# starkware-libs/stark-perpetual

Hardware: AMD Instinct MI355X
Metric: pedersen_hashes_per_sec (higher is better)
Workload: dtype u32x9; 1 GPU; 2^16-leaf Pedersen Merkle rebuild per GPU (BASELINE.json configs[1]), 63 rebuilds in lockstep; tree_height=16, leaves_per_gpu=65536, calls_per_region=28, streams=2, window_bits=26, combine=none

## Files before the change

### stark-perpetual_amd/csrc/curve.hpp

```cpp
#pragma once
#include "fp29.hpp"

namespace sp {

struct aff {
  fe x, y;
};
struct xyzz {
  fe X, Y, ZZ, ZZZ;
};
struct jac {
  fe X, Y, Z;
};

SP_HD xyzz xyzz_from_aff(const aff& p) {
  xyzz r;
  r.X = p.x;
  r.Y = p.y;
  r.ZZ = FE_ONE_M;
  r.ZZZ = FE_ONE_M;
  return r;
}

template <bool SCAN = false>
SP_HD xyzz xyzz_madd(const xyzz& a, const aff& q) {
  if constexpr (SCAN && SP_FE_SCAN) {
    fe t[3];
    fe_scan(t, scan_mul{q.x, a.ZZ}, scan_mul{q.y, a.ZZZ});
    const fe P = fe_sub(t[0], a.X), R = fe_sub(t[1], a.Y);
    const fe P2 = fe_dbl(P), R2 = fe_dbl(R);
    fe_scan(t, scan_sqr{P, P2}, scan_sqr{R, R2});
    const fe PP = t[0], RR = t[1];
    fe_scan(t, scan_mul{P, PP}, scan_mul{a.X, PP});
    const fe PPP = t[0], Q = t[1];
    xyzz r;
    r.X = fe_carry(fe_sub(fe_sub(RR, PPP), fe_dbl(Q)));
    const fe D = fe_sub(Q, r.X), nY = fe_neg_pinned(a.Y);
    fe_scan(t, scan_mul2{R, D, nY, PPP}, scan_mul{a.ZZ, PP}, scan_mul{a.ZZZ, PPP});
    r.Y = t[0];
    r.ZZ = t[1];
    r.ZZZ = t[2];
    return r;
  }
  const fe U2 = fe_mul_t<SCAN>(q.x, a.ZZ);
  const fe S2 = fe_mul_t<SCAN>(q.y, a.ZZZ);
  const fe P = fe_sub(U2, a.X);
  const fe R = fe_sub(S2, a.Y);
  const fe PP = fe_sqr_t<SCAN>(P);
  const fe PPP = fe_mul_t<SCAN>(P, PP);
  const fe Q = fe_mul_t<SCAN>(a.X, PP);
  xyzz r;
  r.X = fe_carry(fe_sub(fe_sub(fe_sqr_t<SCAN>(R), PPP), fe_dbl(Q)));
  r.Y = fe_mul_sub_mul_t<SCAN>(R, fe_sub(Q, r.X), a.Y, PPP);
  r.ZZ = fe_mul_t<SCAN>(a.ZZ, PP);
  r.ZZZ = fe_mul_t<SCAN>(a.ZZZ, PPP);
  return r;
}

template <bool SCAN = false>
SP_HD void xyzz_madd_x_only(const xyzz& a, const aff& q, fe& X3, fe& ZZ3) {
  if constexpr (SCAN && SP_FE_SCAN) {
    fe t[3];
    fe_scan(t, scan_mul{q.x, a.ZZ}, scan_mul{q.y, a.ZZZ});
    const fe P = fe_sub(t[0], a.X), R = fe_sub(t[1], a.Y);
    const fe P2 = fe_dbl(P), R2 = fe_dbl(R);
    fe_scan(t, scan_sqr{P, P2}, scan_sqr{R, R2});
    const fe PP = t[0], RR = t[1];
    fe_scan(t, scan_mul{P, PP}, scan_mul{a.X, PP}, scan_mul{a.ZZ, PP});
    X3 = fe_carry(fe_sub(fe_sub(RR, t[0]), fe_dbl(t[1])));
    ZZ3 = t[2];
    return;
  }
  const fe U2 = fe_mul_t<SCAN>(q.x, a.ZZ);
  const fe S2 = fe_mul_t<SCAN>(q.y, a.ZZZ);
  const fe P = fe_sub(U2, a.X);
  const fe R = fe_sub(S2, a.Y);
  const fe PP = fe_sqr_t<SCAN>(P);
  const fe PPP = fe_mul_t<SCAN>(P, PP);
  const fe Q = fe_mul_t<SCAN>(a.X, PP);
  X3 = fe_carry(fe_sub(fe_sub(fe_sqr_t<SCAN>(R), PPP), fe_dbl(Q)));
  ZZ3 = fe_mul_t<SCAN>(a.ZZ, PP);
}

template <bool SCAN = false>
SP_HD xyzz xyzz_mmadd(const aff& a, const aff& b) {
  if constexpr (SCAN && SP_FE_SCAN) {
    const fe P = fe_sub(b.x, a.x), R = fe_carry(fe_sub(b.y, a.y));
    const fe P2 = fe_dbl(P), R2 = fe_dbl(R);
    fe t[2];
    fe_scan(t, scan_sqr{P, P2}, scan_sqr{R, R2});
    const fe PP = t[0], RR = t[1];
    fe_scan(t, scan_mul{P, PP}, scan_mul{a.x, PP});
    const fe PPP = t[0], Q = t[1];
    xyzz r;
    r.X = fe_carry(fe_sub(fe_sub(RR, PPP), fe_dbl(Q)));
    r.Y = fe_mul_sub_mul_scan(R, fe_sub(Q, r.X), a.y, PPP);
    r.ZZ = PP;
    r.ZZZ = PPP;
    return r;
  }
  const fe P = fe_sub(b.x, a.x);
  const fe R = fe_carry(fe_sub(b.y, a.y));
  const fe PP = fe_sqr_t<SCAN>(P);
  const fe PPP = fe_mul_t<SCAN>(P, PP);
  const fe Q = fe_mul_t<SCAN>(a.x, PP);
  xyzz r;
  r.X = fe_carry(fe_sub(fe_sub(fe_sqr_t<SCAN>(R), PPP), fe_dbl(Q)));
  r.Y = fe_mul_sub_mul_t<SCAN>(R, fe_sub(Q, r.X), a.y, PPP);
  r.ZZ = PP;
  r.ZZZ = PPP;
  return r;
}

template <bool SCAN = false>
SP_HD xyzz xyzz_add(const xyzz& a, const xyzz& b) {
  const fe U1 = fe_mul_t<SCAN>(a.X, b.ZZ);
  const fe U2 = fe_mul_t<SCAN>(b.X, a.ZZ);
  const fe S1 = fe_mul_t<SCAN>(a.Y, b.ZZZ);
  const fe S2 = fe_mul_t<SCAN>(b.Y, a.ZZZ);
  const fe P = fe_sub(U2, U1);
  const fe R = fe_sub(S2, S1);
  const fe PP = fe_sqr_t<SCAN>(P);
  const fe PPP = fe_mul_t<SCAN>(P, PP);
  const fe Q = fe_mul_t<SCAN>(U1, PP);
  xyzz r;
  r.X = fe_carry(fe_sub(fe_sub(fe_sqr_t<SCAN>(R), PPP), fe_dbl(Q)));
  r.Y = fe_mul_sub_mul_t<SCAN>(R, fe_sub(Q, r.X), S1, PPP);
  r.ZZ = fe_mul_t<SCAN>(fe_mul_t<SCAN>(a.ZZ, b.ZZ), PP);
  r.ZZZ = fe_mul_t<SCAN>(fe_mul_t<SCAN>(a.ZZZ, b.ZZZ), PPP);
  return r;
}

template <bool SCAN = false>
SP_HD void xyzz_add_x_only(const xyzz& a, const xyzz& b, fe& X3, fe& ZZ3) {
  const fe U1 = fe_mul_t<SCAN>(a.X, b.ZZ);
  const fe U2 = fe_mul_t<SCAN>(b.X, a.ZZ);
  const fe S1 = fe_mul_t<SCAN>(a.Y, b.ZZZ);
  const fe S2 = fe_mul_t<SCAN>(b.Y, a.ZZZ);
  const fe P = fe_sub(U2, U1);
  const fe R = fe_sub(S2, S1);
  const fe PP = fe_sqr_t<SCAN>(P);
  const fe PPP = fe_mul_t<SCAN>(P, PP);
  const fe Q = fe_mul_t<SCAN>(U1, PP);
  X3 = fe_carry(fe_sub(fe_sub(fe_sqr_t<SCAN>(R), PPP), fe_dbl(Q)));
  ZZ3 = fe_mul_t<SCAN>(fe_mul_t<SCAN>(a.ZZ, b.ZZ), PP);
}

SP_HD jac jac_dbl(const jac& p, const fe& a_coef) {
  const fe XX = fe_sqr(p.X);
  const fe YY = fe_sqr(p.Y);
  const fe YYYY = fe_sqr(YY);
  const fe ZZ = fe_sqr(p.Z);
  const fe t0 = fe_carry(fe_add(p.X, YY));
  const fe halfS = fe_carry(fe_sub(fe_sub(fe_sqr(t0), XX), YYYY));
  const fe S = fe_carry(fe_dbl(halfS));
  const fe XX3 = fe_carry(fe_add(fe_dbl(XX), XX));
// ... 75 lines not shown
```

### stark-perpetual_amd/csrc/fp29.hpp

```cpp
#pragma once
#include <stdint.h>
#include <utility>

#if defined(__HIPCC__)
#include <hip/hip_runtime.h>
#define SP_HD __host__ __device__ __forceinline__
#else
#define SP_HD inline
#endif

#if defined(SP_CHECK_BOUNDS) && !defined(__HIPCC__)
#include <stdio.h>
#include <stdlib.h>
#define SP_CHK32(expr64)                                                        \
  do {                                                                          \
    long long v__ = (long long)(expr64);                                        \
    if (v__ > 2147483647LL || v__ < -2147483648LL) {                            \
      fprintf(stderr, "limb overflow at %s:%d\n", __FILE__, __LINE__);          \
      abort();                                                                  \
    }                                                                           \
  } while (0)
#define SP_CHK64(expr128)                                                       \
  do {                                                                          \
    __int128 v__ = (expr128);                                                   \
// ... 217 lines not shown
  cols t;
  cols_zero(t);
  cols_mac(t, a, b);
  cols_msub(t, c, d);
  return fe_reduce(t);
}
SP_HD fe fe_mul_add_mul(const fe& a, const fe& b, const fe& c, const fe& d) {
  cols t;
  cols_zero(t);
  cols_mac(t, a, b);
  cols_mac(t, c, d);
  return fe_reduce(t);
}

SP_HD fe fe_mul3_add(const fe& a, const fe& b, const fe& c, const fe& d, const fe& e, const fe& f) {
  cols t;
  cols_zero(t);
  cols_mac(t, a, b);
  cols_mac(t, c, d);
  cols_mac(t, e, f);
  return fe_reduce(t);
}

SP_HD void scan_pin(int64_t& acc) {
#if defined(__HIP_DEVICE_COMPILE__)
  asm("" : "+v"(acc));
#else
  (void)acc;
#endif
}
SP_HD void scan_mac(int64_t& acc, int32_t a, int32_t b) {
  SP_CHK64((__int128)acc + (__int128)a * b);
  acc += (int64_t)a * (int64_t)b;
  scan_pin(acc);
}
SP_HD fe fe_neg_pinned(const fe& a) {
  fe r = fe_neg(a);
  fe_pin(r);
  return r;
}
struct scan_mul {
  static constexpr int STEPS = NL;
  const fe &a, &b;
  SP_HD void step(int c, int i, int64_t& acc) const {
    const int j = c - i;
    if (j >= 0 && j < NL) scan_mac(acc, a.l[i], b.l[j]);
// ... 91 lines not shown
  fe_scan(&r, scan_sqr{a, d});
  return r;
}
SP_HD fe fe_mul_sub_mul_scan(const fe& a, const fe& b, const fe& c, const fe& d) {
  const fe nc = fe_neg_pinned(c);
  fe r;
  fe_scan(&r, scan_mul2{a, b, nc, d});
  return r;
}
SP_HD fe fe_mul_add_mul_scan(const fe& a, const fe& b, const fe& c, const fe& d) {
  fe r;
  fe_scan(&r, scan_mul2{a, b, c, d});
  return r;
}
SP_HD fe fe_mul3_add_scan(const fe& a, const fe& b, const fe& c, const fe& d, const fe& e, const fe& f) {
  fe r;
  fe_scan(&r, scan_mul3{a, b, c, d, e, f});
  return r;
}

#ifndef SP_FE_SCAN
#define SP_FE_SCAN 1
#endif
template <bool SCAN>
SP_HD fe fe_mul_t(const fe& a, const fe& b) {
  if constexpr (SCAN && SP_FE_SCAN) return fe_mul_scan(a, b);
  else return fe_mul(a, b);
}
template <bool SCAN>
SP_HD fe fe_sqr_t(const fe& a) {
  if constexpr (SCAN && SP_FE_SCAN) return fe_sqr_scan(a);
  else return fe_sqr(a);
}
template <bool SCAN>
SP_HD fe fe_mul_sub_mul_t(const fe& a, const fe& b, const fe& c, const fe& d) {
  if constexpr (SCAN && SP_FE_SCAN) return fe_mul_sub_mul_scan(a, b, c, d);
  else return fe_mul_sub_mul(a, b, c, d);
}

SP_HD bool fe_geq_p_canon_limbs(const fe& a) {
  const bool gt8 = a.l[8] > P8, eq8 = a.l[8] == P8;
  const bool gt6 = a.l[6] > P6, eq6 = a.l[6] == P6;
  const bool low = (a.l[5] | a.l[4] | a.l[3] | a.l[2] | a.l[1]) != 0 || a.l[0] >= 1;
  return gt8 | (eq8 & ((a.l[7] != 0) | gt6 | (eq6 & low)));
}
SP_HD fe fe_canon(const fe& a_in) {
  fe a;
  {
    const int32_t q = a_in.l[8] >> 19;
    a = a_in;
    a.l[0] -= q;
    a.l[6] -= q * P6;
    a.l[8] -= q * P8;
    a = fe_carry(a);
  }
  const int32_t neg = a.l[8] >> 31;
  a.l[0] += neg & 1;
  a.l[6] += neg & P6;
  a.l[8] += neg & P8;
// ... 594 lines not shown
```

### stark-perpetual_amd/csrc/pedersen.hip

```cpp
#include <algorithm>
#include <cstdlib>
#include <cstring>
#include <map>
#include <vector>

#include "context.hpp"
#include "quad.hpp"

#ifndef SP_ACC_WAVES
#define SP_ACC_WAVES 1
#endif

namespace sp {

struct raw_aff {
  u256 x, y;
};
__device__ __forceinline__ raw_aff ld_raw(const aff_packed* e) {
  const uint4* q = reinterpret_cast<const uint4*>(e);
  const uint4 a = q[0], b = q[1], c = q[2], d = q[3];
  raw_aff r;
  r.x.w[0] = a.x; r.x.w[1] = a.y; r.x.w[2] = a.z; r.x.w[3] = a.w;
  r.x.w[4] = b.x; r.x.w[5] = b.y; r.x.w[6] = b.z; r.x.w[7] = b.w;
  r.y.w[0] = c.x; r.y.w[1] = c.y; r.y.w[2] = c.z; r.y.w[3] = c.w;
// ... 66 lines not shown
#pragma unroll
  for (int k = 0; k < NL; ++k) v.l[k] = base[(size_t)k * n + e];
  return v;
}

__device__ __forceinline__ void operand_pointers(const uint64_t* x, const uint64_t* y, size_t xstride,
                                                 size_t ystride, const int2* __restrict__ src, size_t e,
                                                 const uint64_t*& fx, const uint64_t*& fy) {
  if (src == nullptr) {
    fx = x + 4 * e * xstride;
    fy = y + 4 * e * ystride;
  } else {
    const int2 s = src[e];
    fx = s.x >= 0 ? x + 4 * (size_t)s.x : y;
    fy = s.y >= 0 ? x + 4 * (size_t)s.y : y;
  }
}

#ifndef SP_SCAN_BULK
#define SP_SCAN_BULK true
#endif
#ifndef SP_SCAN_SPLIT
#define SP_SCAN_SPLIT false
#endif

__device__ __forceinline__ void
bulk_accumulate(const uint64_t* __restrict__ x, const uint64_t* __restrict__ y, size_t xstride,
                size_t ystride, size_t n, const aff_packed* __restrict__ ped, int w0, int log2e,
                int nwin, int32_t* __restrict__ sX, int32_t* __restrict__ sZZ,
                uint8_t* __restrict__ status, unsigned* __restrict__ flag,
                const int2* __restrict__ src, size_t plane, size_t e) {
  if (e >= n) return;
  const uint64_t *fx, *fy;
  operand_pointers(x, y, xstride, ystride, src, e, fx, fy);
  u256 sx = ld_u256(fx);
  u256 sy = ld_u256(fy);
  uint8_t st = SP_HASH_OK;
  if (!u256_lt(sx, U256_P) || !u256_lt(sy, U256_P)) {
    st = SP_HASH_OUT_OF_RANGE;
#pragma unroll
    for (int i = 0; i < 8; ++i) { sx.w[i] = 0; sy.w[i] = 0; }
  }
  bits512 str = concat_xy(sx, sy);
  auto next_window = [&](int g) {
    return window_entry(ped, g, pop_bits(str, window_width(g, w0, log2e)), w0, log2e);
  };
// ... 62 lines not shown
}

__device__ __forceinline__ fe shfl_xor_fe(const fe& v, int mask) {
  fe r;
#pragma unroll
  for (int i = 0; i < NL; ++i) r.l[i] = __shfl_xor(v.l[i], mask, 64);
  return r;
}
__device__ __forceinline__ uint32_t field_from_memory(const uint64_t* felt, int bit, int width) {
  const uint32_t* w = reinterpret_cast<const uint32_t*>(felt);
  const int wi = bit >> 5, sh = bit & 31;
  uint64_t two = (uint64_t)w[wi];
  if (wi + 1 < 8) two |= (uint64_t)w[wi + 1] << 32;
  return (uint32_t)(two >> sh) & ((1u << width) - 1u);
}
__device__ __forceinline__ uint32_t window_from_memory(const uint64_t* fx, const uint64_t* fy, int start,
                                                       int width) {
  if (start + width <= 252) return field_from_memory(fx, start, width);
  if (start >= 252) return field_from_memory(fy, start - 252, width);
  const int lo_n = 252 - start;
  return field_from_memory(fx, start, lo_n) | (field_from_memory(fy, 0, width - lo_n) << lo_n);
}

template <int LOG_L>
__device__ __forceinline__ xyzz split_accumulate(const uint64_t* fx, const uint64_t* fy, int sub,
                                                 const aff_packed* __restrict__ ped, int w0, int log2e,
                                                 int nwin) {
  constexpr int L = 1 << LOG_L;
  const int cnt_lo = nwin / L, extra = nwin % L;
  const int cnt = cnt_lo + (sub < extra ? 1 : 0);
  const int g0 = sub * cnt_lo + (sub < extra ? sub : extra);
  auto entry = [&](int g) {
    return window_entry(ped, g, window_from_memory(fx, fy, window_start(g, w0, log2e), window_width(g, w0, log2e)),
                        w0, log2e);
  };
  const window_ref r0 = entry(g0);
  const aff q0 = signed_aff(ld_raw(r0.entry), r0.negative);
  window_ref rn = entry(g0 + 1);
  raw_aff nxt = ld_raw(rn.entry);
  xyzz acc;
  {
    const aff q1 = signed_aff(nxt, rn.negative);
    if (cnt > 2) {
      rn = entry(g0 + 2);
      nxt = ld_raw(rn.entry);
    }
    acc = xyzz_mmadd<SP_SCAN_SPLIT>(q0, q1);
  }
  for (int j = 2; j < cnt; ++j) {
    const aff q = signed_aff(nxt, rn.negative);
    if (j + 1 < cnt) {
      rn = entry(g0 + j + 1);
      nxt = ld_raw(rn.entry);
    }
    acc = xyzz_madd<SP_SCAN_SPLIT>(acc, q);
  }
#pragma unroll 1
  for (int r = 0; r + 1 < LOG_L; ++r) {
    xyzz o;
    o.X = shfl_xor_fe(acc.X, 1 << r);
    o.Y = shfl_xor_fe(acc.Y, 1 << r);
    o.ZZ = shfl_xor_fe(acc.ZZ, 1 << r);
    o.ZZZ = shfl_xor_fe(acc.ZZZ, 1 << r);
    acc = xyzz_add<SP_SCAN_SPLIT>(acc, o);
  }
  if constexpr (LOG_L > 0) {
    constexpr int r = LOG_L - 1;
    xyzz o;
    o.X = shfl_xor_fe(acc.X, 1 << r);
    o.Y = shfl_xor_fe(acc.Y, 1 << r);
    o.ZZ = shfl_xor_fe(acc.ZZ, 1 << r);
    o.ZZZ = shfl_xor_fe(acc.ZZZ, 1 << r);
    fe X3, ZZ3;
    xyzz_add_x_only<SP_SCAN_SPLIT>(acc, o, X3, ZZ3);
    acc.X = X3;
    acc.ZZ = ZZ3;
  }
  return acc;
}

template <int LOG_L, bool FUSED>
__global__ void __launch_bounds__(256)
ped_accumulate_split_kernel(const uint64_t* __restrict__ x, const uint64_t* __restrict__ y, size_t xstride,
                            size_t ystride, size_t n, const aff_packed* __restrict__ ped, int w0, int log2e,
                            int nwin, int32_t* __restrict__ sX, int32_t* __restrict__ sZZ,
                            uint8_t* __restrict__ status, unsigned* __restrict__ flag,
                            const int2* __restrict__ src, uint64_t* __restrict__ out, size_t ostride,
                            size_t plane) {
  constexpr int L = 1 << LOG_L;
  const size_t gt = (size_t)blockIdx.x * blockDim.x + threadIdx.x;
  const size_t e_raw = gt >> LOG_L;
  const int sub = (int)(gt & (L - 1));
  const bool active = e_raw < n;
  const size_t e = active ? e_raw : n - 1;
  const uint64_t *fx, *fy;
  operand_pointers(x, y, xstride, ystride, src, e, fx, fy);
  const xyzz acc = split_accumulate<LOG_L>(fx, fy, sub, ped, w0, log2e, nwin);
  uint8_t st = SP_HASH_OK;
  u256 xa_plain;
  if (FUSED) {
    fe zz = acc.ZZ;
    if constexpr (LOG_L < 2) {
      if (fe_is_zero(zz)) {
        zz = FE_ONE_M;
        st = SP_HASH_UNHASHABLE;
      }
    }
    const fe zinv = fe_inv_shared_quad<(LOG_L >= 2 ? 0 : 2 - LOG_L), true>(zz, (int)(threadIdx.x & 3));
    if constexpr (LOG_L >= 2) {
      if (limbs_is_zero(zinv)) st = SP_HASH_UNHASHABLE;
    }
    xa_plain = fe_pack(fe_canon(fe_mul(acc.X, zinv)));
  }
  if (!active || sub != 0) return;
  if (!u256_lt(ld_u256(fx), U256_P) || !u256_lt(ld_u256(fy), U256_P)) st = SP_HASH_OUT_OF_RANGE;
  if (FUSED) {
    st_u256(out + 4 * e * ostride, xa_plain);
  } else {
    store_limbs(sX, plane, e, acc.X);
    store_limbs(sZZ, plane, e, acc.ZZ);
  }
  if (status) status[e] = st;
  if (st != SP_HASH_OK && flag) atomicOr(flag, (unsigned)st);
}

template <int LOG_L>
__global__ void __launch_bounds__(256, SP_ACC_WAVES)
ped_accumulate_mixed_kernel(const uint64_t* __restrict__ x, const uint64_t* __restrict__ y, size_t xstride,
                            size_t ystride, size_t n_bulk, size_t rem, unsigned bulk_blocks,
                            const aff_packed* __restrict__ ped, int w0, int log2e, int nwin,
                            int32_t* __restrict__ sX, int32_t* __restrict__ sZZ, uint8_t* __restrict__ status,
                            unsigned* __restrict__ flag, const int2* __restrict__ src, size_t plane) {
  if (blockIdx.x < bulk_blocks) {
    bulk_accumulate(x, y, xstride, ystride, n_bulk, ped, w0, log2e, nwin, sX, sZZ, status, flag, src, plane,
                    (size_t)blockIdx.x * blockDim.x + threadIdx.x);
    return;
  }
  constexpr int L = 1 << LOG_L;
  const size_t gt = (size_t)(blockIdx.x - bulk_blocks) * blockDim.x + threadIdx.x;
  const size_t e_raw = gt >> LOG_L;
  const int sub = (int)(gt & (L - 1));
  const bool active = e_raw < rem;
  const size_t e = n_bulk + (active ? e_raw : rem - 1);
  const uint64_t *fx, *fy;
  operand_pointers(x, y, xstride, ystride, src, e, fx, fy);
  const xyzz acc = split_accumulate<LOG_L>(fx, fy, sub, ped, w0, log2e, nwin);
  if (!active || sub != 0) return;
  uint8_t st = SP_HASH_OK;
  if (!u256_lt(ld_u256(fx), U256_P) || !u256_lt(ld_u256(fy), U256_P)) st = SP_HASH_OUT_OF_RANGE;
  store_limbs(sX, plane, e, acc.X);
  store_limbs(sZZ, plane, e, acc.ZZ);
  if (status) status[e] = st;
  if (st != SP_HASH_OK && flag) atomicOr(flag, (unsigned)st);
}

template <int LOG_Q, bool SPARSE>
__device__ __forceinline__ u256 quad_hash(const uint64_t* fx, const uint64_t* fy, int mode, const aff_packed* __restrict__ cpts,
                                          int cx, int cy, const aff_packed* __restrict__ ped, int w0, int log2e,
                                          int nwin_plan, int g, bool* unhashable) {
  constexpr int QUADS = 1 << LOG_Q;
  const int q = g >> 2, k = g & 3;
  int nwin = nwin_plan, first_real = 0;
  if constexpr (SPARSE) {
    nwin = mode == 0 ? nwin_plan : 1 + nwin_plan - (mode == 1 ? cx : cy);
    first_real = mode == 1 ? cx - 1 : (mode == 2 ? -1 : 0);
  }
  auto entry = [&](int v) {
    if constexpr (SPARSE) {
      if (mode != 0 && v == 0) return unpack_raw(ld_raw(cpts + (mode - 1)));
// ... 27 lines not shown
    s.b = fe_dpp<quad_perm(0, 1, 0, 1)>(p.b);
  }
  for (int j = 4; j < max_cnt; ++j) {
    const aff pj = entry(j < cnt ? q + j * QUADS : q);
    qpt t;
    t.a = fe_sel(upper, odd ? pj.y : pj.x, s.a);
    t.b = fe_sel(upper, FE_ONE_M, s.b);
    const qpt u = qadd<false>(t, k);
    if (j < cnt) s = u;
  }
#define SP_BUTTERFLY(XORV, LAST)                               \
  {                                                            \
    qpt t;                                                     \
    t.a = fe_sel(upper, fe_swizzle_xor<XORV>(s.a), s.a);       \
    t.b = fe_sel(upper, fe_swizzle_xor<XORV>(s.b), s.b);       \
    s = qadd<LAST>(t, k);                                      \
  }
  if constexpr (LOG_Q == 1) SP_BUTTERFLY(4, true)
  if constexpr (LOG_Q == 2) { SP_BUTTERFLY(4, false) SP_BUTTERFLY(8, true) }
  if constexpr (LOG_Q == 3) { SP_BUTTERFLY(4, false) SP_BUTTERFLY(8, false) SP_BUTTERFLY(16, true) }
#undef SP_BUTTERFLY
  const fe zinv = fe_inv_quad<true>(s.b, k);
  *unhashable = limbs_is_zero(zinv);
  return fe_pack(fe_canon(fe_mul(s.a, zinv)));
}

template <int LOG_Q, bool SPARSE = false>
__global__ void __launch_bounds__(256)
ped_quad_kernel(const uint64_t* __restrict__ x, const uint64_t* __restrict__ y, size_t xstride, size_t ystride,
                size_t n, const aff_packed* __restrict__ ped, int w0, int log2e, int nwin_plan,
                uint8_t* __restrict__ status, unsigned* __restrict__ flag, const int2* __restrict__ src,
                uint64_t* __restrict__ out, size_t ostride, int dup, const aff_packed* __restrict__ cpts, int cx,
                int cy) {
  constexpr int QUADS = 1 << LOG_Q, LANES = 4 * QUADS;
  const size_t gt = (size_t)blockIdx.x * blockDim.x + threadIdx.x;
  const size_t e_raw = gt / ((size_t)LANES << dup);
  const int g = (int)(gt % LANES);
  const bool active = e_raw < n;
  const size_t e = active ? e_raw : n - 1;
  const uint64_t *fx, *fy;
  operand_pointers(x, y, xstride, ystride, src, e, fx, fy);
  int mode = 0;
  if constexpr (SPARSE) {
    const int2 sc = src[e];
    mode = sc.x < 0 ? 1 : (sc.y < 0 ? 2 : 0);
  }
  bool unhashable;
// ... 208 lines not shown
    }
    __syncthreads();
    out += 4 * n_out;
    n_out >>= 1;
  }
}

__global__ void __launch_bounds__(256)
ped_finish_kernel(const int32_t* __restrict__ sX, int32_t* __restrict__ sZZ, int32_t* __restrict__ sPre,
                  size_t n, size_t T, uint64_t* __restrict__ out, size_t ostride,
                  uint8_t* __restrict__ status, unsigned* __restrict__ flag) {
  const size_t t = (size_t)blockIdx.x * blockDim.x + threadIdx.x;
  if (t >= T) return;
  const size_t cnt = t < n ? (n - t + T - 1) / T : 0;
  fe run = FE_ONE_M;
  if (cnt > 0) {
    fe znext = load_limbs(sZZ, n, t);
#pragma unroll 1
    for (size_t j = 0; j < cnt; ++j) {
      const size_t e = t + j * T;
      const fe z = znext;
      if (j + 1 < cnt) znext = load_limbs(sZZ, n, e + T);
      store_limbs(sPre, n, e, run);
      run = fe_mul(run, z);
    }
  }
  if (fe_is_zero(run)) {
    run = FE_ONE_M;
#pragma unroll 1
    for (size_t e = t; e < n; e += T) {
      fe z = load_limbs(sZZ, n, e);
      if (fe_is_zero(z)) {
        z = FE_ONE_M;
        store_limbs(sZZ, n, e, z);
        if (status) status[e] = SP_HASH_UNHASHABLE;
        if (flag) atomicOr(flag, (unsigned)SP_HASH_UNHASHABLE);
      }
      store_limbs(sPre, n, e, run);
      run = fe_mul(run, z);
    }
  }
  size_t e = cnt > 0 ? t + (cnt - 1) * T : 0;
  fe zn = run, pn = run, xn = run;
  if (cnt > 0) {
    zn = load_limbs(sZZ, n, e);
    pn = load_limbs(sPre, n, e);
    xn = load_limbs(sX, n, e);
  }
  fe inv = fe_inv_shared_quad<2, true>(run, (int)(threadIdx.x & 3));
#pragma unroll 1
  for (size_t j = cnt; j-- > 0;) {
    const fe z = zn, pre = pn, xv = xn;
    const size_t cur = t + j * T;
    if (j > 0) {
      zn = load_limbs(sZZ, n, cur - T);
      pn = load_limbs(sPre, n, cur - T);
      xn = load_limbs(sX, n, cur - T);
    }
    const fe zinv = fe_mul(inv, pre);
    inv = fe_mul(inv, z);
    const fe xa = fe_mul(xv, zinv);
    st_u256(out + 4 * cur * ostride, fe_pack(fe_canon(xa)));
  }
}

template <bool Z_IN_LDS>
__global__ void __launch_bounds__(256)
ped_finish_lds_kernel(const int32_t* __restrict__ sX, int32_t* __restrict__ sZZ, size_t n, size_t T,
                      uint64_t* __restrict__ out, size_t ostride, uint8_t* __restrict__ status,
                      unsigned* __restrict__ flag, int kmax) {
  extern __shared__ int32_t fin_lds[];
  int32_t* lpre = fin_lds;
  int32_t* lz = fin_lds + (size_t)kmax * NL * 256;
  auto lds_put = [&](int32_t* base, size_t j, const fe& v) {
#pragma unroll
    for (int k = 0; k < NL; ++k) base[((j * NL + k) << 8) + threadIdx.x] = v.l[k];
  };
  auto lds_get = [&](const int32_t* base, size_t j) {
    fe v;
#pragma unroll
    for (int k = 0; k < NL; ++k) v.l[k] = base[((j * NL + k) << 8) + threadIdx.x];
    return v;
  };
  const size_t t = (size_t)blockIdx.x * blockDim.x + threadIdx.x;
  if (t >= T) return;
  const size_t cnt = t < n ? (n - t + T - 1) / T : 0;
  fe run = FE_ONE_M;
  if (cnt > 0) {
    fe znext = load_limbs(sZZ, n, t);
#pragma unroll 1
    for (size_t j = 0; j < cnt; ++j) {
      const fe z = znext;
      if (j + 1 < cnt) znext = load_limbs(sZZ, n, t + (j + 1) * T);
      lds_put(lpre, j, run);
      if (Z_IN_LDS) lds_put(lz, j, z);
      run = fe_mul(run, z);
    }
  }
  if (fe_is_zero(run)) {
    run = FE_ONE_M;
    size_t j = 0;
#pragma unroll 1
    for (size_t e = t; e < n; e += T, ++j) {
      fe z = load_limbs(sZZ, n, e);
      if (fe_is_zero(z)) {
        z = FE_ONE_M;
        store_limbs(sZZ, n, e, z);
        if (status) status[e] = SP_HASH_UNHASHABLE;
        if (flag) atomicOr(flag, (unsigned)SP_HASH_UNHASHABLE);
      }
      lds_put(lpre, j, run);
      if (Z_IN_LDS) lds_put(lz, j, z);
      run = fe_mul(run, z);
    }
  }
  size_t e = cnt > 0 ? t + (cnt - 1) * T : 0;
  fe zn = run, xn = run;
  if (cnt > 0) {
    if (!Z_IN_LDS) zn = load_limbs(sZZ, n, e);
    xn = load_limbs(sX, n, e);
  }
  fe inv = fe_inv_shared_quad<2, true>(run, (int)(threadIdx.x & 3));
#pragma unroll 1
  for (size_t j = cnt; j-- > 0;) {
    const fe z = Z_IN_LDS ? lds_get(lz, j) : zn, xv = xn;
    const fe pre = lds_get(lpre, j);
    const size_t cur = t + j * T;
    if (j > 0) {
      if (!Z_IN_LDS) zn = load_limbs(sZZ, n, cur - T);
      xn = load_limbs(sX, n, cur - T);
    }
    const fe zinv = fe_mul(inv, pre);
    inv = fe_mul(inv, z);
    const fe xa = fe_mul(xv, zinv);
    st_u256(out + 4 * cur * ostride, fe_pack(fe_canon(xa)));
  }
}

__global__ void __launch_bounds__(128)
ped_point_kernel(const uint64_t* __restrict__ x, const uint64_t* __restrict__ y, size_t n,
                 const aff_packed* __restrict__ ped, int w0, int log2e, int nwin,
                 uint64_t* __restrict__ ox, uint64_t* __restrict__ oy, uint8_t* __restrict__ status) {
  size_t e = (size_t)blockIdx.x * blockDim.x + threadIdx.x;
  if (e >= n) e = n - 1;
  u256 sx = ld_u256(x + 4 * e);
  u256 sy = ld_u256(y + 4 * e);
  if (!u256_lt(sx, U256_P) || !u256_lt(sy, U256_P)) {
    status[e] = SP_HASH_OUT_OF_RANGE;
    return;
  }
  bits512 str = concat_xy(sx, sy);
  xyzz acc = xyzz_from_aff(ld_aff(ped + pop_bits(str, w0)));
  for (int g = 1; g < nwin; ++g) {
    const window_ref r = window_entry(ped, g, pop_bits(str, log2e + 1), w0, log2e);
    acc = xyzz_madd(acc, signed_aff(ld_raw(r.entry), r.negative));
  }
  if (fe_is_zero(acc.ZZ)) {
// ... 5 lines not shown
  st_u256(oy + 4 * e, fe_pack(fe_from_mont(fe_mul(acc.Y, izzz))));
  status[e] = SP_HASH_OK;
}

__global__ void __launch_bounds__(64)
ped_partial_kernel(const uint64_t* __restrict__ felts, int count, const aff_packed* __restrict__ ped, int w0, int log2e,
                   int nwin, int cx, int cy, aff_packed* __restrict__ out) {
  int t = (int)(blockIdx.x * blockDim.x + threadIdx.x);
  if (t >= 2 * count) t = 2 * count - 1;
  const int side = t & 1;
  const uint64_t* f = felts + 4 * (size_t)(t >> 1);
  const int g0 = side == 0 ? 0 : nwin - cy, g1 = side == 0 ? cx : nwin;
  auto entry = [&](int w) {
    const window_ref r =
        window_entry(ped, w, window_from_memory(f, f, window_start(w, w0, log2e), window_width(w, w0, log2e)), w0, log2e);
    return signed_aff(ld_raw(r.entry), r.negative);
  };
  aff_packed res;
  if (g1 - g0 == 1) {
    const aff a = entry(g0);
    res.x = fe_pack(fe_canon(a.x));
    res.y = fe_pack(fe_canon(a.y));
  } else {
    xyzz acc = xyzz_mmadd(entry(g0), entry(g0 + 1));
    for (int g = g0 + 2; g < g1; ++g) acc = xyzz_madd(acc, entry(g));
    const fe izzz = fe_inv(acc.ZZZ);
    const fe izz = fe_sqr(fe_mul(acc.ZZ, izzz));
    res.x = fe_pack(fe_canon(fe_mul(acc.X, izz)));
    res.y = fe_pack(fe_canon(fe_mul(acc.Y, izzz)));
  }
  uint4* q = reinterpret_cast<uint4*>(out + t);
  q[0] = make_uint4(res.x.w[0], res.x.w[1], res.x.w[2], res.x.w[3]);
  q[1] = make_uint4(res.x.w[4], res.x.w[5], res.x.w[6], res.x.w[7]);
  q[2] = make_uint4(res.y.w[0], res.y.w[1], res.y.w[2], res.y.w[3]);
  q[3] = make_uint4(res.y.w[4], res.y.w[5], res.y.w[6], res.y.w[7]);
}

struct KernelProfile {
  bool enabled = false;
  std::vector<hipEvent_t> ev;
  std::vector<size_t> units;
  size_t used = 0;
};
static KernelProfile g_prof;
static bool g_split_enabled = getenv("STARKPERP_NO_SPLIT") == nullptr;
static bool g_fuse_enabled = getenv("STARKPERP_NO_FUSE") == nullptr;
static bool g_quad_enabled = getenv("STARKPERP_NO_QUAD") == nullptr;
static bool g_quad2_enabled = getenv("STARKPERP_NO_QUAD2") == nullptr;
static bool g_level_split = getenv("STARKPERP_NO_LEVEL_SPLIT") == nullptr;
static bool g_quad_no_dup = getenv("STARKPERP_QUAD_NO_DUP") != nullptr;
static bool g_sparse_enabled = getenv("STARKPERP_NO_SPARSE_LEVELS") == nullptr;
static size_t g_quad_max = getenv("STARKPERP_QUAD_MAX") ? (size_t)atoll(getenv("STARKPERP_QUAD_MAX")) : 2048;
// ... 764 lines not shown
```

### stark-perpetual_amd/csrc/quad.hpp

```cpp
#pragma once
#include "curve.hpp"

namespace sp {

constexpr int quad_perm(int a, int b, int c, int d) { return a | (b << 2) | (c << 4) | (d << 6); }

template <int CTRL>
__device__ __forceinline__ fe fe_dpp(const fe& v) {
  fe r;
#pragma unroll
  for (int i = 0; i < NL; ++i) {
    r.l[i] = __builtin_amdgcn_mov_dpp(v.l[i], CTRL, 0xF, 0xF, true);
    asm volatile("" : "+v"(r.l[i]));
  }
  return r;
}
template <int XOR>
__device__ __forceinline__ fe fe_swizzle_xor(const fe& v) {
  fe r;
#pragma unroll
  for (int i = 0; i < NL; ++i) r.l[i] = __builtin_amdgcn_ds_swizzle(v.l[i], (XOR << 10) | 0x1F);
  return r;
}
__device__ __forceinline__ fe fe_sel(bool c, const fe& a, const fe& b) {
  fe r;
#pragma unroll
  for (int i = 0; i < NL; ++i) r.l[i] = c ? a.l[i] : b.l[i];
  return r;
}

struct qpt {
  fe a, b;
};

template <bool X_ONLY>
__device__ __forceinline__ qpt qadd(const qpt& p, int k) {
  const bool h = (k & 2) != 0, e = (k & 1) != 0;
  const fe T1 = fe_mul(p.a, fe_dpp<quad_perm(2, 3, 0, 1)>(p.b));
  const fe D = fe_sub(fe_dpp<quad_perm(2, 3, 0, 1)>(T1), T1);
  const fe T2 = fe_mul(fe_sel(h, p.b, D), fe_sel(h, fe_dpp<quad_perm(0, 1, 0, 1)>(p.b), D));
  const fe PPb = fe_dpp<quad_perm(0, 0, 0, 0)>(T2);
  const fe l3 = fe_sel(k == 0, D, fe_sel(k == 1, fe_dpp<quad_perm(0, 0, 0, 0)>(T1), T2));
  const fe r3 = fe_sel(k == 3, fe_dpp<quad_perm(0, 0, 0, 0)>(D), PPb);
  const fe T3 = fe_mul(l3, r3);
  const fe Qb = fe_dpp<quad_perm(1, 1, 1, 1)>(T3);
  const fe X3 =
      fe_carry(fe_sub(fe_sub(fe_dpp<quad_perm(1, 1, 1, 1)>(T2), fe_dpp<quad_perm(0, 0, 0, 0)>(T3)), fe_dbl(Qb)));
  qpt r;
  if (X_ONLY) {
    r.a = X3;
    r.b = fe_dpp<quad_perm(2, 2, 2, 2)>(T3);
    return r;
  }
  const fe l4 = fe_sel(k == 0, fe_dpp<quad_perm(1, 1, 1, 1)>(T1), fe_sel(k == 1, D, T3));
  const fe r4 = fe_sel(k == 1, fe_sub(T3, X3), fe_sel(k == 3, PPb, T3));
  const fe T4 = fe_mul(l4, r4);
  const fe Y3 = fe_sub(fe_dpp<quad_perm(1, 1, 1, 1)>(T4), fe_dpp<quad_perm(0, 0, 0, 0)>(T4));
  r.a = fe_sel(e, Y3, X3);
  r.b = fe_sel(e, fe_dpp<quad_perm(3, 3, 3, 3)>(T4), fe_dpp<quad_perm(2, 2, 2, 2)>(T3));
  return r;
}

__device__ __forceinline__ qpt qmmadd(const fe& x1, const fe& y1, const fe& x2, const fe& y2, int k) {
  const bool e = (k & 1) != 0;
  const fe P = fe_sub(x2, x1), R = fe_carry(fe_sub(y2, y1));
  const fe T1 = fe_sqr(fe_sel(e, R, P));
  const fe PPb = fe_dpp<quad_perm(0, 0, 2, 2)>(T1);
  const fe T2 = fe_mul(fe_sel(e, x1, P), PPb);
  const fe PPPb = fe_dpp<quad_perm(0, 0, 2, 2)>(T2), Qb = fe_dpp<quad_perm(1, 1, 3, 3)>(T2);
  const fe X3 = fe_carry(fe_sub(fe_sub(fe_dpp<quad_perm(1, 1, 3, 3)>(T1), PPPb), fe_dbl(Qb)));
  const fe T3 = fe_mul(fe_sel(e, R, y1), fe_sel(e, fe_sub(Qb, X3), PPPb));
  const fe Y3 = fe_sub(fe_dpp<quad_perm(1, 1, 3, 3)>(T3), fe_dpp<quad_perm(0, 0, 2, 2)>(T3));
  qpt r;
  r.a = fe_sel(e, Y3, X3);
  r.b = fe_sel(e, PPPb, PPb);
  return r;
}

__device__ __forceinline__ void quad_gcd_update(fe& own, const trans2x2& t, int k) {
  const bool odd = (k & 1) != 0, modular = (k & 2) != 0;
  const fe par = fe_dpp<quad_perm(1, 0, 3, 2)>(own);
  const int32_t co = odd ? t.r : t.u, cp = odd ? t.q : t.v;
  const int64_t a = co, b = cp;
  const int32_t so = own.l[NL - 1] >> 31, sp_ = par.l[NL - 1] >> 31;
  int32_t m = (co & so) + (cp & sp_);
  int64_t c = a * own.l[0] + b * par.l[0];
  m -= (int32_t)(((uint32_t)c + (uint32_t)m) & LMASK);
  m = modular ? m : 0;
  c += m;
  c >>= LB;
  fe r;
#pragma unroll
  for (int i = 1; i < NL; ++i) {
    c += a * own.l[i] + b * par.l[i];
// ... 59 lines not shown
    ad = f64_dpp<quad_perm(0, 0, 0, 0)>(od);
    const double bd = f64_dpp<quad_perm(1, 1, 1, 1)>(od);
    lehmer_rows m;
    ok &= lehmer_batch(__builtin_fabs(ad), __builtin_fabs(bd), m);
    if (__all(bd == 0.0 || !ok)) break;
    const double co = odd ? lehmer_flip(m.vb, bd) : lehmer_flip(m.ua, ad);
    const double cp = odd ? lehmer_flip(m.ub, ad) : lehmer_flip(m.va, bd);
    own = lehmer_row(own, fe_dpp<quad_perm(1, 0, 3, 2)>(own), (int32_t)co, (int32_t)cp);
  }
  {
    const double od = lehmer_to_double(own);
    ad = f64_dpp<quad_perm(0, 0, 0, 0)>(od);
    ok &= f64_dpp<quad_perm(1, 1, 1, 1)>(od) == 0.0;
  }
  if (__any(!ok)) {
    return fe_inv_plain_quad_divsteps(fe_canon(fe_mul(x, FE_ONE_M)), k);
  }
  const fe d = __builtin_fabs(ad) == 1.0 ? fe_dpp<quad_perm(2, 2, 2, 2)>(own) : FE_ZERO;
  return lehmer_finish(d, ad < 0.0 ? -1 : 0);
}

template <bool PLAIN = false>
__device__ __forceinline__ fe fe_inv_quad(const fe& a, int k) {
  return fe_mul(fe_inv_plain_quad(a, k), PLAIN ? FE_R2 : FE_R3);
}


template <int LOG_DISTINCT, bool PLAIN = false>
__device__ __forceinline__ fe fe_inv_shared_quad(const fe& a, int k) {
  if constexpr (LOG_DISTINCT == 0) {
    return fe_inv_quad<PLAIN>(a, k);
  } else if constexpr (LOG_DISTINCT == 1) {
    const fe other = fe_dpp<quad_perm(2, 3, 0, 1)>(a);
    const fe pinv = fe_inv_quad<PLAIN>(fe_mul(a, other), k);
    return fe_mul(pinv, other);
  } else {
    const fe nb = fe_dpp<quad_perm(1, 0, 3, 2)>(a);
    const fe pair = fe_mul(a, nb);
    const fe opp = fe_dpp<quad_perm(2, 3, 0, 1)>(pair);
    const fe pinv = fe_inv_quad<PLAIN>(fe_mul(pair, opp), k);
    return fe_mul(pinv, fe_mul(nb, opp));
  }
}

}
```

Measured before the change: 1.044 billion hashes/s.

## Add rotating-SGPR-carry multiply form and use it in split accumulation

Adds a third field-multiply form that issues v_mad_i64_i32 through inline asm. The carry outputs rotate across a small pool of scalar registers, so the compiler no longer has to allocate and serialize them. The field multiply template is widened from a bool to an int form selector. The split-accumulate path now defaults to this rotating form, while the finish and quad paths keep the existing column form behind macros. The aim is fewer register and dependency stalls in the 9x9 limb multiply-accumulate. The risk is that the hand-pinned asm limits compiler scheduling or raises SGPR pressure.

```diff
diff --git a/stark-perpetual_amd/csrc/curve.hpp b/stark-perpetual_amd/csrc/curve.hpp
--- a/stark-perpetual_amd/csrc/curve.hpp
+++ b/stark-perpetual_amd/csrc/curve.hpp
@@ -22,9 +22,9 @@
   return r;
 }
 
-template <bool SCAN = false>
+template <int SCAN = FE_COLS>
 SP_HD xyzz xyzz_madd(const xyzz& a, const aff& q) {
-  if constexpr (SCAN && SP_FE_SCAN) {
+  if constexpr (SCAN == FE_SCAN && SP_FE_SCAN) {
     fe t[3];
     fe_scan(t, scan_mul{q.x, a.ZZ}, scan_mul{q.y, a.ZZZ});
     const fe P = fe_sub(t[0], a.X), R = fe_sub(t[1], a.Y);
@@ -57,9 +57,9 @@
   return r;
 }
 
-template <bool SCAN = false>
+template <int SCAN = FE_COLS>
 SP_HD void xyzz_madd_x_only(const xyzz& a, const aff& q, fe& X3, fe& ZZ3) {
-  if constexpr (SCAN && SP_FE_SCAN) {
+  if constexpr (SCAN == FE_SCAN && SP_FE_SCAN) {
     fe t[3];
     fe_scan(t, scan_mul{q.x, a.ZZ}, scan_mul{q.y, a.ZZZ});
     const fe P = fe_sub(t[0], a.X), R = fe_sub(t[1], a.Y);
@@ -82,9 +82,9 @@
   ZZ3 = fe_mul_t<SCAN>(a.ZZ, PP);
 }
 
-template <bool SCAN = false>
+template <int SCAN = FE_COLS>
 SP_HD xyzz xyzz_mmadd(const aff& a, const aff& b) {
-  if constexpr (SCAN && SP_FE_SCAN) {
+  if constexpr (SCAN == FE_SCAN && SP_FE_SCAN) {
     const fe P = fe_sub(b.x, a.x), R = fe_carry(fe_sub(b.y, a.y));
     const fe P2 = fe_dbl(P), R2 = fe_dbl(R);
     fe t[2];
@@ -112,7 +112,7 @@
   return r;
 }
 
-template <bool SCAN = false>
+template <int SCAN = FE_COLS>
 SP_HD xyzz xyzz_add(const xyzz& a, const xyzz& b) {
   const fe U1 = fe_mul_t<SCAN>(a.X, b.ZZ);
   const fe U2 = fe_mul_t<SCAN>(b.X, a.ZZ);
@@ -131,7 +131,7 @@
   return r;
 }
 
-template <bool SCAN = false>
+template <int SCAN = FE_COLS>
 SP_HD void xyzz_add_x_only(const xyzz& a, const xyzz& b, fe& X3, fe& ZZ3) {
   const fe U1 = fe_mul_t<SCAN>(a.X, b.ZZ);
   const fe U2 = fe_mul_t<SCAN>(b.X, a.ZZ);
diff --git a/stark-perpetual_amd/csrc/fp29.hpp b/stark-perpetual_amd/csrc/fp29.hpp
--- a/stark-perpetual_amd/csrc/fp29.hpp
+++ b/stark-perpetual_amd/csrc/fp29.hpp
@@ -263,6 +263,110 @@
   return fe_reduce(t);
 }
 
+#ifndef SP_MAC_ROTATE
+#define SP_MAC_ROTATE 1
+#endif
+constexpr int MAC_SLOTS = 8;
+constexpr int MAC_DIST = 3;
+#if defined(__HIP_DEVICE_COMPILE__) && SP_MAC_ROTATE
+#define SP_MAC_ROTATE_DEVICE 1
+struct mac_sink {
+  uint64_t s[MAC_SLOTS];
+  int n;
+};
+__device__ __forceinline__ void mac_open(mac_sink& k) {
+#pragma unroll
+  for (int i = 0; i < MAC_SLOTS; ++i) asm volatile("" : "=s"(k.s[i]));
+  k.n = 0;
+}
+__device__ __forceinline__ void mac_done(mac_sink& k) {
+  asm volatile("" ::"s"(k.s[0]), "s"(k.s[1]), "s"(k.s[2]), "s"(k.s[3]), "s"(k.s[4]), "s"(k.s[5]), "s"(k.s[6]), "s"(k.s[7]));
+}
+__device__ __forceinline__ void mac_rot(mac_sink& k, int64_t& acc, int32_t a, int32_t b, bool first) {
+  uint64_t& co = k.s[k.n++ % MAC_SLOTS];
+  if (first) asm volatile("v_mad_i64_i32 %0, %1, %2, %3, 0" : "=&v"(acc), "+s"(co) : "v"(a), "v"(b));
+  else asm volatile("v_mad_i64_i32 %0, %1, %2, %3, %0" : "+v"(acc), "+s"(co) : "v"(a), "v"(b));
+}
+__device__ __forceinline__ void mac_rot_s(mac_sink& k, int64_t& acc, int32_t a, int32_t b) {
+  uint64_t& co = k.s[k.n++ % MAC_SLOTS];
+  asm volatile("v_mad_i64_i32 %0, %1, %2, %3, %0" : "+v"(acc), "+s"(co) : "v"(a), "s"(b));
+}
+__device__ __forceinline__ void cols_mac_rot(mac_sink& k, cols& t, const fe& a, const fe& b, bool fresh) {
+#pragma unroll
+  for (int i = 0; i < NL; ++i)
+#pragma unroll
+    for (int j = 0; j < NL; ++j) mac_rot(k, t.c[i + j], a.l[i], b.l[j], fresh && (i == 0 || j == NL - 1));
+}
+__device__ __forceinline__ void cols_sqr_rot(mac_sink& k, cols& t, const fe& a) {
+  const fe d2 = fe_dbl(a);
+#pragma unroll
+  for (int d = 0; d < NL; ++d)
+#pragma unroll
+    for (int i = 0; i + d < NL; ++i) mac_rot(k, t.c[2 * i + d], d == 0 ? a.l[i] : d2.l[i], a.l[i + d], d < 2);
+}
+__device__ __forceinline__ fe fe_reduce_rot(mac_sink& k, cols& t) {
+  int32_t np6 = -P6, np8 = -P8;
+  asm volatile("" : "+s"(np6), "+s"(np8));
+#pragma unroll
+  for (int i = 0; i < NL; ++i) {
+    const int32_t q = (int32_t)((uint32_t)t.c[i] & LMASK);
+    t.c[i + 1] += t.c[i] >> LB;
+    mac_rot_s(k, t.c[i + 6], q, np6);
+    mac_rot_s(k, t.c[i + 8], q, np8);
+  }
+  mac_done(k);
+  fe r;
+  int64_t carry = 0;
+#pragma unroll
+  for (int j = 0; j < 8; ++j) {
+    const int64_t v = t.c[9 + j] + carry;
+    r.l[j] = (int32_t)((uint32_t)v & LMASK);
+    carry = v >> LB;
+  }
+  r.l[8] = (int32_t)carry;
+  fe_pin(r);
+  return r;
+}
+#else
+#define SP_MAC_ROTATE_DEVICE 0
+#endif
+SP_HD fe fe_mul_rot(const fe& a, const fe& b) {
+#if SP_MAC_ROTATE_DEVICE
+  mac_sink k;
+  cols t;
+  mac_open(k);
+  cols_mac_rot(k, t, a, b, true);
+  return fe_reduce_rot(k, t);
+#else
+  return fe_mul(a, b);
+#endif
+}
+SP_HD fe fe_sqr_rot(const fe& a) {
+#if SP_MAC_ROTATE_DEVICE
+  mac_sink k;
+  cols t;
+  mac_open(k);
+  cols_sqr_rot(k, t, a);
+  return fe_reduce_rot(k, t);
+#else
+  return fe_sqr(a);
+#endif
+}
+SP_HD fe fe_mul_sub_mul_rot(const fe& a, const fe& b, const fe& c, const fe& d) {
+#if SP_MAC_ROTATE_DEVICE
+  mac_sink k;
+  cols t;
+  fe nc = fe_neg(c);
+  fe_pin(nc);
+  mac_open(k);
+  cols_mac_rot(k, t, a, b, true);
+  cols_mac_rot(k, t, nc, d, false);
+  return fe_reduce_rot(k, t);
+#else
+  return fe_mul_sub_mul(a, b, c, d);
+#endif
+}
+
 SP_HD void scan_pin(int64_t& acc) {
 #if defined(__HIP_DEVICE_COMPILE__)
   asm("" : "+v"(acc));
@@ -400,19 +504,23 @@
 #ifndef SP_FE_SCAN
 #define SP_FE_SCAN 1
 #endif
-template <bool SCAN>
+constexpr int FE_COLS = 0, FE_SCAN = 1, FE_ROT = 2;
+template <int FORM>
 SP_HD fe fe_mul_t(const fe& a, const fe& b) {
-  if constexpr (SCAN && SP_FE_SCAN) return fe_mul_scan(a, b);
+  if constexpr (FORM == FE_SCAN && SP_FE_SCAN) return fe_mul_scan(a, b);
+  else if constexpr (FORM == FE_ROT) return fe_mul_rot(a, b);
   else return fe_mul(a, b);
 }
-template <bool SCAN>
+template <int FORM>
 SP_HD fe fe_sqr_t(const fe& a) {
-  if constexpr (SCAN && SP_FE_SCAN) return fe_sqr_scan(a);
+  if constexpr (FORM == FE_SCAN && SP_FE_SCAN) return fe_sqr_scan(a);
+  else if constexpr (FORM == FE_ROT) return fe_sqr_rot(a);
   else return fe_sqr(a);
 }
-template <bool SCAN>
+template <int FORM>
 SP_HD fe fe_mul_sub_mul_t(const fe& a, const fe& b, const fe& c, const fe& d) {
-  if constexpr (SCAN && SP_FE_SCAN) return fe_mul_sub_mul_scan(a, b, c, d);
+  if constexpr (FORM == FE_SCAN && SP_FE_SCAN) return fe_mul_sub_mul_scan(a, b, c, d);
+  else if constexpr (FORM == FE_ROT) return fe_mul_sub_mul_rot(a, b, c, d);
   else return fe_mul_sub_mul(a, b, c, d);
 }
 
diff --git a/stark-perpetual_amd/csrc/pedersen.hip b/stark-perpetual_amd/csrc/pedersen.hip
--- a/stark-perpetual_amd/csrc/pedersen.hip
+++ b/stark-perpetual_amd/csrc/pedersen.hip
@@ -112,6 +112,12 @@
 #endif
 #ifndef SP_SCAN_SPLIT
 #define SP_SCAN_SPLIT false
+#endif
+#ifndef SP_FORM_SPLIT
+#define SP_FORM_SPLIT FE_ROT
+#endif
+#ifndef SP_FORM_FINISH
+#define SP_FORM_FINISH FE_COLS
 #endif
 
 __device__ __forceinline__ void
@@ -220,7 +226,7 @@
   return field_from_memory(fx, start, lo_n) | (field_from_memory(fy, 0, width - lo_n) << lo_n);
 }
 
-template <int LOG_L>
+template <int LOG_L, int FORM>
 __device__ __forceinline__ xyzz split_accumulate(const uint64_t* fx, const uint64_t* fy, int sub,
                                                  const aff_packed* __restrict__ ped, int w0, int log2e,
                                                  int nwin) {
@@ -243,7 +249,7 @@
       rn = entry(g0 + 2);
       nxt = ld_raw(rn.entry);
     }
-    acc = xyzz_mmadd<SP_SCAN_SPLIT>(q0, q1);
+    acc = xyzz_mmadd<FORM>(q0, q1);
   }
   for (int j = 2; j < cnt; ++j) {
     const aff q = signed_aff(nxt, rn.negative);
@@ -251,7 +257,7 @@
       rn = entry(g0 + j + 1);
       nxt = ld_raw(rn.entry);
     }
-    acc = xyzz_madd<SP_SCAN_SPLIT>(acc, q);
+    acc = xyzz_madd<FORM>(acc, q);
   }
 #pragma unroll 1
   for (int r = 0; r + 1 < LOG_L; ++r) {
@@ -260,7 +266,7 @@
     o.Y = shfl_xor_fe(acc.Y, 1 << r);
     o.ZZ = shfl_xor_fe(acc.ZZ, 1 << r);
     o.ZZZ = shfl_xor_fe(acc.ZZZ, 1 << r);
-    acc = xyzz_add<SP_SCAN_SPLIT>(acc, o);
+    acc = xyzz_add<FORM>(acc, o);
   }
   if constexpr (LOG_L > 0) {
     constexpr int r = LOG_L - 1;
@@ -270,7 +276,7 @@
     o.ZZ = shfl_xor_fe(acc.ZZ, 1 << r);
     o.ZZZ = shfl_xor_fe(acc.ZZZ, 1 << r);
     fe X3, ZZ3;
-    xyzz_add_x_only<SP_SCAN_SPLIT>(acc, o, X3, ZZ3);
+    xyzz_add_x_only<FORM>(acc, o, X3, ZZ3);
     acc.X = X3;
     acc.ZZ = ZZ3;
   }
@@ -293,7 +299,7 @@
   const size_t e = active ? e_raw : n - 1;
   const uint64_t *fx, *fy;
   operand_pointers(x, y, xstride, ystride, src, e, fx, fy);
-  const xyzz acc = split_accumulate<LOG_L>(fx, fy, sub, ped, w0, log2e, nwin);
+  const xyzz acc = split_accumulate<LOG_L, SP_FORM_SPLIT>(fx, fy, sub, ped, w0, log2e, nwin);
   uint8_t st = SP_HASH_OK;
   u256 xa_plain;
   if (FUSED) {
@@ -308,7 +314,7 @@
     if constexpr (LOG_L >= 2) {
       if (limbs_is_zero(zinv)) st = SP_HASH_UNHASHABLE;
     }
-    xa_plain = fe_pack(fe_canon(fe_mul(acc.X, zinv)));
+    xa_plain = fe_pack(fe_canon(fe_mul_t<SP_FORM_SPLIT>(acc.X, zinv)));
   }
   if (!active || sub != 0) return;
   if (!u256_lt(ld_u256(fx), U256_P) || !u256_lt(ld_u256(fy), U256_P)) st = SP_HASH_OUT_OF_RANGE;
@@ -342,7 +348,7 @@
   const size_t e = n_bulk + (active ? e_raw : rem - 1);
   const uint64_t *fx, *fy;
   operand_pointers(x, y, xstride, ystride, src, e, fx, fy);
-  const xyzz acc = split_accumulate<LOG_L>(fx, fy, sub, ped, w0, log2e, nwin);
+  const xyzz acc = split_accumulate<LOG_L, SP_SCAN_SPLIT>(fx, fy, sub, ped, w0, log2e, nwin);
   if (!active || sub != 0) return;
   uint8_t st = SP_HASH_OK;
   if (!u256_lt(ld_u256(fx), U256_P) || !u256_lt(ld_u256(fy), U256_P)) st = SP_HASH_OUT_OF_RANGE;
@@ -416,7 +422,7 @@
 #undef SP_BUTTERFLY
   const fe zinv = fe_inv_quad<true>(s.b, k);
   *unhashable = limbs_is_zero(zinv);
-  return fe_pack(fe_canon(fe_mul(s.a, zinv)));
+  return fe_pack(fe_canon(fe_mul_t<SP_FORM_QUAD>(s.a, zinv)));
 }
 
 template <int LOG_Q, bool SPARSE = false>
@@ -671,7 +677,7 @@
       const fe z = znext;
       if (j + 1 < cnt) znext = load_limbs(sZZ, n, e + T);
       store_limbs(sPre, n, e, run);
-      run = fe_mul(run, z);
+      run = fe_mul_t<SP_FORM_FINISH>(run, z);
     }
   }
   if (fe_is_zero(run)) {
@@ -686,7 +692,7 @@
         if (flag) atomicOr(flag, (unsigned)SP_HASH_UNHASHABLE);
       }
       store_limbs(sPre, n, e, run);
-      run = fe_mul(run, z);
+      run = fe_mul_t<SP_FORM_FINISH>(run, z);
     }
   }
   size_t e = cnt > 0 ? t + (cnt - 1) * T : 0;
@@ -706,9 +712,9 @@
       pn = load_limbs(sPre, n, cur - T);
       xn = load_limbs(sX, n, cur - T);
     }
-    const fe zinv = fe_mul(inv, pre);
-    inv = fe_mul(inv, z);
-    const fe xa = fe_mul(xv, zinv);
+    const fe zinv = fe_mul_t<SP_FORM_FINISH>(inv, pre);
+    inv = fe_mul_t<SP_FORM_FINISH>(inv, z);
+    const fe xa = fe_mul_t<SP_FORM_FINISH>(xv, zinv);
     st_u256(out + 4 * cur * ostride, fe_pack(fe_canon(xa)));
   }
 }
@@ -743,7 +749,7 @@
       if (j + 1 < cnt) znext = load_limbs(sZZ, n, t + (j + 1) * T);
       lds_put(lpre, j, run);
       if (Z_IN_LDS) lds_put(lz, j, z);
-      run = fe_mul(run, z);
+      run = fe_mul_t<SP_FORM_FINISH>(run, z);
     }
   }
   if (fe_is_zero(run)) {
@@ -760,7 +766,7 @@
       }
       lds_put(lpre, j, run);
       if (Z_IN_LDS) lds_put(lz, j, z);
-      run = fe_mul(run, z);
+      run = fe_mul_t<SP_FORM_FINISH>(run, z);
     }
   }
   size_t e = cnt > 0 ? t + (cnt - 1) * T : 0;
@@ -779,9 +785,9 @@
       if (!Z_IN_LDS) zn = load_limbs(sZZ, n, cur - T);
       xn = load_limbs(sX, n, cur - T);
     }
-    const fe zinv = fe_mul(inv, pre);
-    inv = fe_mul(inv, z);
-    const fe xa = fe_mul(xv, zinv);
+    const fe zinv = fe_mul_t<SP_FORM_FINISH>(inv, pre);
+    inv = fe_mul_t<SP_FORM_FINISH>(inv, z);
+    const fe xa = fe_mul_t<SP_FORM_FINISH>(xv, zinv);
     st_u256(out + 4 * cur * ostride, fe_pack(fe_canon(xa)));
   }
 }
@@ -833,12 +839,12 @@
     res.x = fe_pack(fe_canon(a.x));
     res.y = fe_pack(fe_canon(a.y));
   } else {
-    xyzz acc = xyzz_mmadd(entry(g0), entry(g0 + 1));
-    for (int g = g0 + 2; g < g1; ++g) acc = xyzz_madd(acc, entry(g));
+    xyzz acc = xyzz_mmadd<SP_FORM_FINISH>(entry(g0), entry(g0 + 1));
+    for (int g = g0 + 2; g < g1; ++g) acc = xyzz_madd<SP_FORM_FINISH>(acc, entry(g));
     const fe izzz = fe_inv(acc.ZZZ);
-    const fe izz = fe_sqr(fe_mul(acc.ZZ, izzz));
-    res.x = fe_pack(fe_canon(fe_mul(acc.X, izz)));
-    res.y = fe_pack(fe_canon(fe_mul(acc.Y, izzz)));
+    const fe izz = fe_sqr_t<SP_FORM_FINISH>(fe_mul_t<SP_FORM_FINISH>(acc.ZZ, izzz));
+    res.x = fe_pack(fe_canon(fe_mul_t<SP_FORM_FINISH>(acc.X, izz)));
+    res.y = fe_pack(fe_canon(fe_mul_t<SP_FORM_FINISH>(acc.Y, izzz)));
   }
   uint4* q = reinterpret_cast<uint4*>(out + t);
   q[0] = make_uint4(res.x.w[0], res.x.w[1], res.x.w[2], res.x.w[3]);
diff --git a/stark-perpetual_amd/csrc/quad.hpp b/stark-perpetual_amd/csrc/quad.hpp
--- a/stark-perpetual_amd/csrc/quad.hpp
+++ b/stark-perpetual_amd/csrc/quad.hpp
@@ -2,6 +2,10 @@
 #include "curve.hpp"
 
 namespace sp {
+
+#ifndef SP_FORM_QUAD
+#define SP_FORM_QUAD FE_COLS
+#endif
 
 constexpr int quad_perm(int a, int b, int c, int d) { return a | (b << 2) | (c << 4) | (d << 6); }
 
@@ -36,13 +40,13 @@
 template <bool X_ONLY>
 __device__ __forceinline__ qpt qadd(const qpt& p, int k) {
   const bool h = (k & 2) != 0, e = (k & 1) != 0;
-  const fe T1 = fe_mul(p.a, fe_dpp<quad_perm(2, 3, 0, 1)>(p.b));
+  const fe T1 = fe_mul_t<SP_FORM_QUAD>(p.a, fe_dpp<quad_perm(2, 3, 0, 1)>(p.b));
   const fe D = fe_sub(fe_dpp<quad_perm(2, 3, 0, 1)>(T1), T1);
-  const fe T2 = fe_mul(fe_sel(h, p.b, D), fe_sel(h, fe_dpp<quad_perm(0, 1, 0, 1)>(p.b), D));
+  const fe T2 = fe_mul_t<SP_FORM_QUAD>(fe_sel(h, p.b, D), fe_sel(h, fe_dpp<quad_perm(0, 1, 0, 1)>(p.b), D));
   const fe PPb = fe_dpp<quad_perm(0, 0, 0, 0)>(T2);
   const fe l3 = fe_sel(k == 0, D, fe_sel(k == 1, fe_dpp<quad_perm(0, 0, 0, 0)>(T1), T2));
   const fe r3 = fe_sel(k == 3, fe_dpp<quad_perm(0, 0, 0, 0)>(D), PPb);
-  const fe T3 = fe_mul(l3, r3);
+  const fe T3 = fe_mul_t<SP_FORM_QUAD>(l3, r3);
   const fe Qb = fe_dpp<quad_perm(1, 1, 1, 1)>(T3);
   const fe X3 =
       fe_carry(fe_sub(fe_sub(fe_dpp<quad_perm(1, 1, 1, 1)>(T2), fe_dpp<quad_perm(0, 0, 0, 0)>(T3)), fe_dbl(Qb)));
@@ -54,7 +58,7 @@
   }
   const fe l4 = fe_sel(k == 0, fe_dpp<quad_perm(1, 1, 1, 1)>(T1), fe_sel(k == 1, D, T3));
   const fe r4 = fe_sel(k == 1, fe_sub(T3, X3), fe_sel(k == 3, PPb, T3));
-  const fe T4 = fe_mul(l4, r4);
+  const fe T4 = fe_mul_t<SP_FORM_QUAD>(l4, r4);
   const fe Y3 = fe_sub(fe_dpp<quad_perm(1, 1, 1, 1)>(T4), fe_dpp<quad_perm(0, 0, 0, 0)>(T4));
   r.a = fe_sel(e, Y3, X3);
   r.b = fe_sel(e, fe_dpp<quad_perm(3, 3, 3, 3)>(T4), fe_dpp<quad_perm(2, 2, 2, 2)>(T3));
@@ -64,12 +68,12 @@
 __device__ __forceinline__ qpt qmmadd(const fe& x1, const fe& y1, const fe& x2, const fe& y2, int k) {
   const bool e = (k & 1) != 0;
   const fe P = fe_sub(x2, x1), R = fe_carry(fe_sub(y2, y1));
-  const fe T1 = fe_sqr(fe_sel(e, R, P));
+  const fe T1 = fe_sqr_t<SP_FORM_QUAD>(fe_sel(e, R, P));
   const fe PPb = fe_dpp<quad_perm(0, 0, 2, 2)>(T1);
-  const fe T2 = fe_mul(fe_sel(e, x1, P), PPb);
+  const fe T2 = fe_mul_t<SP_FORM_QUAD>(fe_sel(e, x1, P), PPb);
   const fe PPPb = fe_dpp<quad_perm(0, 0, 2, 2)>(T2), Qb = fe_dpp<quad_perm(1, 1, 3, 3)>(T2);
   const fe X3 = fe_carry(fe_sub(fe_sub(fe_dpp<quad_perm(1, 1, 3, 3)>(T1), PPPb), fe_dbl(Qb)));
-  const fe T3 = fe_mul(fe_sel(e, R, y1), fe_sel(e, fe_sub(Qb, X3), PPPb));
+  const fe T3 = fe_mul_t<SP_FORM_QUAD>(fe_sel(e, R, y1), fe_sel(e, fe_sub(Qb, X3), PPPb));
   const fe Y3 = fe_sub(fe_dpp<quad_perm(1, 1, 3, 3)>(T3), fe_dpp<quad_perm(0, 0, 2, 2)>(T3));
   qpt r;
   r.a = fe_sel(e, Y3, X3);
@@ -175,7 +179,7 @@
 
 template <bool PLAIN = false>
 __device__ __forceinline__ fe fe_inv_quad(const fe& a, int k) {
-  return fe_mul(fe_inv_plain_quad(a, k), PLAIN ? FE_R2 : FE_R3);
+  return fe_mul_t<SP_FORM_QUAD>(fe_inv_plain_quad(a, k), PLAIN ? FE_R2 : FE_R3);
 }
 
 
@@ -185,15 +189,15 @@
     return fe_inv_quad<PLAIN>(a, k);
   } else if constexpr (LOG_DISTINCT == 1) {
     const fe other = fe_dpp<quad_perm(2, 3, 0, 1)>(a);
-    const fe pinv = fe_inv_quad<PLAIN>(fe_mul(a, other), k);
-    return fe_mul(pinv, other);
+    const fe pinv = fe_inv_quad<PLAIN>(fe_mul_t<SP_FORM_QUAD>(a, other), k);
+    return fe_mul_t<SP_FORM_QUAD>(pinv, other);
   } else {
     const fe nb = fe_dpp<quad_perm(1, 0, 3, 2)>(a);
-    const fe pair = fe_mul(a, nb);
+    const fe pair = fe_mul_t<SP_FORM_QUAD>(a, nb);
     const fe opp = fe_dpp<quad_perm(2, 3, 0, 1)>(pair);
-    const fe pinv = fe_inv_quad<PLAIN>(fe_mul(pair, opp), k);
-    return fe_mul(pinv, fe_mul(nb, opp));
-  }
-}
-
-}
+    const fe pinv = fe_inv_quad<PLAIN>(fe_mul_t<SP_FORM_QUAD>(pair, opp), k);
+    return fe_mul_t<SP_FORM_QUAD>(pinv, fe_mul_t<SP_FORM_QUAD>(nb, opp));
+  }
+}
+
+}
```

Measured after the change: 1.044 billion hashes/s, median of 2. No clear change (-0.0%).
